# gunesevitan/otto-multi-objective-recommender-system

Hardware: AMD Instinct MI355X
Metric: aid-pairs/sec covisitation build (higher is better)
Workload: dtype u64

## Files before the change

otto-multi-objective-recommender-system_amd/csrc/otto_covis.hip:

```cpp
#include "common.h"
#include "topk.h"
#include "scan.h"
#include "../../include/otto_covis.h"

#include <stdarg.h>
#include <string.h>
#include <type_traits>
#include <vector>

namespace otto {

static thread_local std::string g_err;
void set_error(const char* fmt, ...) {
    char buf[1024];
    va_list ap;
    va_start(ap, fmt);
    vsnprintf(buf, sizeof buf, fmt, ap);
    va_end(ap);
    g_err = buf;
}

struct WinPairs {
    const int64_t* off;
    int W;
// ... 1015 lines not shown
                wave_topk_push(best[j], lb, k);
            }
        }
    }
}

template <int NW, int GATHER_U, typename FB>
__device__ __forceinline__ void for_each_record_batch(const uint64_t* sorted_desc, const uint32_t* rec, uint64_t r0, uint64_t r1,
                                                      int wid, FB fb) {
    const unsigned lane = lane_id();
    const uint32_t l = lane & 31u;
    const int half = (int)(lane >> 5);
    if (r0 >= r1) return;
    auto load_desc = [&](uint64_t cb) {
        const uint64_t mine = cb + (uint64_t)lane * NW + wid;
        return mine < r1 ? sorted_desc[mine] : 0ull;
    };
    uint64_t d = load_desc(r0);
    for (uint64_t cb = r0; cb < r1; cb += (uint64_t)NW * 64) {
        const uint64_t cbn = cb + (uint64_t)NW * 64;
        const uint64_t dn = cbn < r1 ? load_desc(cbn) : 0ull;
        const uint64_t left = r1 - cb;
        const int nrun = left >= (uint64_t)NW * 64 ? 64 : (int)((left + NW - 1 - wid) / NW);
        uint32_t rcA[GATHER_U], rcB[GATHER_U];
        uint64_t slA[GATHER_U], slB[GATHER_U];
        bool okA[GATHER_U], okB[GATHER_U];
        auto issue = [&](int t, uint32_t (&rc)[GATHER_U], uint64_t (&sl)[GATHER_U], bool (&ok)[GATHER_U]) {
#pragma unroll
            for (int u = 0; u < GATHER_U; ++u) {
                const int src = t + 2 * u + half;
                const uint64_t dd = (uint64_t)__shfl((unsigned long long)d, src & 63, 64);
                const uint32_t sp = desc_sp(dd);
                const uint64_t s0 = desc_slot(dd);
                ok[u] = src < 64 && l < desc_len(dd) && l != sp;
                rc[u] = ok[u] ? rec[s0 + l] : 0u;
                sl[u] = s0 + (sp != DESC_SP_NONE ? sp : l);
            }
        };
        auto consume = [&](uint32_t (&rc)[GATHER_U], uint64_t (&sl)[GATHER_U], bool (&ok)[GATHER_U]) { fb(rc, sl, ok); };
        if (nrun > 0) issue(0, rcA, slA, okA);
        for (int t = 0; t < nrun; t += 4 * GATHER_U) {
            const bool hasB = t + 2 * GATHER_U < nrun;
            if (hasB) issue(t + 2 * GATHER_U, rcB, slB, okB);
            consume(rcA, slA, okA);
            if (t + 4 * GATHER_U < nrun) issue(t + 4 * GATHER_U, rcA, slA, okA);
            if (hasB) consume(rcB, slB, okB);
        }
        d = dn;
    }
}

template <int NW, int GATHER_U, bool NEED_SL, typename FB>
__device__ __forceinline__ void for_each_record_seg(const uint64_t* sorted_desc, const uint32_t* rec, uint64_t r0, uint64_t r1,
                                                    int wid, uint8_t* s_seg, FB fb, const uint64_t* d0p = nullptr) {
    const unsigned lane = lane_id();
    const uint32_t g = lane >> 3, gl4 = (lane & 7u) << 2;
    if (r0 >= r1) return;
    auto load_desc = [&](uint64_t cb) {
        const uint64_t mine = cb + (uint64_t)lane * NW + wid;
        return mine < r1 ? sorted_desc[mine] : 0ull;
    };
    uint64_t d = d0p ? *d0p : load_desc(r0);
    for (uint64_t cb = r0; cb < r1; cb += (uint64_t)NW * 64) {
        const uint64_t cbn = cb + (uint64_t)NW * 64;
        const uint64_t dn = cbn < r1 ? load_desc(cbn) : 0ull;
        const uint32_t len = desc_len(d);
        const uint32_t segs = (len + 7u) >> 3;
        const uint32_t incl = wave_incl_scan(segs), excl = incl - segs;
        const uint32_t total = (uint32_t)__builtin_amdgcn_readlane((int)incl, 63);
#pragma unroll
        for (uint32_t k = 0; k < 4; ++k)
            if (k < segs) s_seg[excl + k] = (uint8_t)((lane << 2) | k);
        wave_lds_sync();
        const int nstep = (int)((total + 7u) >> 3);
        const uint64_t recb = (uint64_t)(uintptr_t)rec;
        const uint64_t pre = (recb + (desc_slot(d) << 2)) | ((uint64_t)desc_len(d) << 50) | ((uint64_t)desc_sp(d) << 58);
        const int plo = (int)(uint32_t)pre, phi = (int)(uint32_t)(pre >> 32);
        uint32_t rcA[GATHER_U], rcB[GATHER_U];
        uint64_t slA[NEED_SL ? GATHER_U : 1], slB[NEED_SL ? GATHER_U : 1];
        uint64_t okA[GATHER_U], okB[GATHER_U];
        constexpr int ICMP_NE = 33, ICMP_ULT = 36, ICMP_SLT = 40;
        auto issue = [&](int t, uint32_t (&rc)[GATHER_U], uint64_t (&sl)[NEED_SL ? GATHER_U : 1], uint64_t (&ok)[GATHER_U]) {
            const uint32_t qb = (uint32_t)t * 8u + g;
            const int lim = (int)total - 8 * t;
#pragma unroll
            for (int u = 0; u < GATHER_U; ++u) {
                const uint32_t r = (uint32_t)s_seg[qb + 8u * u];
                const int src = (int)(r & 0xFCu);
                const uint32_t lo = (uint32_t)__builtin_amdgcn_ds_bpermute(src, plo);
                const uint32_t hi = (uint32_t)__builtin_amdgcn_ds_bpermute(src, phi);
                const uint32_t off4 = ((r & 3u) << 5) | gl4;
                const uint32_t len4 = (hi >> 16) & 0xFFu, sp4 = hi >> 24;
                const uint64_t base = ((uint64_t)(hi & 0xFFFFu) << 32) | lo;
                if (NEED_SL) sl[NEED_SL ? u : 0] = (base - recb + (sp4 != DESC_SP_NONE * 4u ? sp4 : off4)) >> 2;
                ok[u] = __builtin_amdgcn_sicmp((int)g, lim - 8 * u, ICMP_SLT) & __builtin_amdgcn_uicmp(off4, len4, ICMP_ULT) &
                        __builtin_amdgcn_uicmp(off4, sp4, ICMP_NE);
                rc[u] = *reinterpret_cast<const __attribute__((address_space(1))) uint32_t*>((uintptr_t)(base + off4));
            }
        };
        if (nstep > 0) issue(0, rcA, slA, okA);
        for (int t = 0; t < nstep; t += 2 * GATHER_U) {
            const bool hasB = t + GATHER_U < nstep;
            if (hasB) issue(t + GATHER_U, rcB, slB, okB);
            fb(rcA, slA, okA);
            if (t + 2 * GATHER_U < nstep) issue(t + 2 * GATHER_U, rcA, slA, okA);
            if (hasB) fb(rcB, slB, okB);
        }
        wave_lds_sync();
        d = dn;
    }
}

template <int NW, int GATHER_U, typename F>
__device__ __forceinline__ void for_each_record(const uint64_t* sorted_desc, const uint32_t* rec, uint64_t r0, uint64_t r1,
                                                int wid, F f) {
    for_each_record_batch<NW, GATHER_U>(sorted_desc, rec, r0, r1, wid,
                                        [&](uint32_t (&rc)[GATHER_U], uint64_t (&sl)[GATHER_U], bool (&ok)[GATHER_U]) {
#pragma unroll
        for (int u = 0; u < GATHER_U; ++u)
            if (ok[u]) f(rc[u], sl[u]);
    });
}

__device__ __forceinline__ uint32_t rec_hash(uint32_t rc) { return (rc & REC_AID_MASK) * 0x9E3779B1u; }

struct PartArgs {
    const uint64_t* chunks;
    uint32_t n_chunks;
    const uint64_t* cnt64;
    const uint8_t* boost;
    const uint64_t* run_start;
    const uint64_t* sorted_desc;
    const uint32_t* rec;
    const uint32_t* tw;
    const uint64_t* litem_start;
    uint32_t* pcount;
    uint32_t* pcursor;
    const uint64_t* pstart;
    uint32_t* prec;
    uint32_t* ptw;
    uint32_t l_cap;
    int window_max;
    int allow_packed;
    uint32_t* flag;
    uint32_t* ovf_count;
    uint32_t* work;
};

__host__ __device__ __forceinline__ uint64_t bucket_cap(uint64_t n_records, int lgR) {
    return lgR == 0 ? 0ull : 2ull * ((n_records + (1ull << lgR) - 1ull) >> lgR) + 256ull;
}
struct ItemCap {
    const uint64_t* items;
// ... 343 lines not shown
            ord[r] = (uint32_t)s;
            for (uint64_t p = 1; p < items; ++p) ord[a.n_pilots[mode] + sm + p - r - 1] = (uint32_t)(s + p);
            const uint64_t cs = run[9] + ex_c;
            for (uint64_t q = 0; q < nch; ++q) a.chunks[cs + q] = (uint64_t)x | (q << 26);
        }
        run[0] += tot_small & 0xFFF;
        run[1] += (tot_small >> 12) & 0xFFF;
        run[2] += tot_l;
#pragma unroll
        for (int m = 0; m < 3; ++m) {
            run[6 + m] += (tot_small >> (24 + 12 * m)) & 0xFFF;
            run[3 + m] += tot_m[m];
        }
        run[9] += tot_c;
    }
}

constexpr uint64_t TAB_EMPTY = ~0ull;

struct ItemDesc {
    uint32_t it;
    uint64_t item;
    uint64_t rb, re;
    uint64_t ps, pe;
};

#ifdef OTTO_PHASE_PROF
#define OTTO_PH(i) do { if (threadIdx.x == 0) { const unsigned long long _t = clock64(); ph[i] += _t - ph_t; ph_t = _t; } } while (0)
#else
#define OTTO_PH(i) do {} while (0)
#endif
template <int LOG2T, int THREADS, int GROUP, bool PACKED, int MINW, int GU, int INS_CH, bool DBG>
__global__ __launch_bounds__(THREADS, MINW) void k_reduce(ReduceArgs a) {
    constexpr int T = 1 << LOG2T;
    constexpr int NW = THREADS / 64;
    constexpr bool TP = GROUP == OTTO_COVIS_GROUP_TIME && PACKED;
    using K = typename std::conditional<GROUP == OTTO_COVIS_GROUP_TIME && !PACKED, KeyW, KeyN>::type;
    constexpr bool WIDE = GROUP == OTTO_COVIS_GROUP_TIME && !PACKED;
    auto kw = [](K key) -> uint64_t { if constexpr (TP) return key.c >> REC_AID_BITS; else return kweight(key); };
    constexpr bool DYNAMIC = true;
    constexpr int EXCAP = 64;
    constexpr int PKD = GROUP == OTTO_COVIS_GROUP_TIME ? 1 : PK;
    constexpr bool BOUND = GROUP == OTTO_COVIS_GROUP_TYPE && PKD > 1 && NW == 1;
    constexpr int CCAP = 256;
    constexpr bool HOT = NW > 1 && GROUP == OTTO_COVIS_GROUP_TYPE;
    __shared__ uint64_t s_tab[PACKED ? T : 1];
    __shared__ uint32_t s_key[PACKED ? 1 : T];
    __shared__ uint32_t s_v[3][PACKED ? 1 : T];
    constexpr int OCAP = NW == 1 ? 1 : (LOG2T == 12 ? 1920 : (LOG2T == 14 ? 10240 : (THREADS == 512 ? 4608 : 6144)));
    constexpr int RCAP = OCAP / NW;
    __shared__ uint16_t s_occ[OCAP];
    __shared__ uint32_t s_wcnt[NW];
    __shared__ uint32_t s_hcnt[NW];
    __shared__ uint16_t s_lbi[NW > 1 ? PKD : 1][NW > 1 ? THREADS : 1];
    __shared__ uint64_t s_exw[(NW > 1 || BOUND) ? PKD : 1][(NW > 1 || BOUND) ? EXCAP : 1];
    __shared__ uint16_t s_cand[BOUND ? CCAP : 1];
    __shared__ uint32_t s_exy[1][(NW > 1 && WIDE) ? EXCAP : 1];
    __shared__ uint64_t s_thrw[PK];
    __shared__ uint32_t s_thry[PK];
    __shared__ uint32_t s_nex[PK];
    __shared__ uint32_t s_more;
    __shared__ uint32_t s_ovf;
    constexpr int LISTCAP = BOUND ? S_CAP : 256;
    __shared__ uint16_t s_list[NW == 1 ? LISTCAP : 1];
    __shared__ uint8_t s_seg[NW * 256 + 32];
    __shared__ ItemDesc s_cur;
    __shared__ ItemDesc s_nxt;

    const int wid = threadIdx.x >> 6;
    const unsigned lane = lane_id();
#ifdef OTTO_PHASE_PROF
    unsigned long long ph[16] = {0, 0, 0, 0, 0, 0, 0, 0, 0, 0, 0, 0, 0, 0, 0, 0}, ph_t = clock64();
#endif

    auto fetch_item = [&](uint32_t idx, ItemDesc& d) {
        d.it = 0xFFFFFFFFu;
        d.item = 0ull;
        if (idx < a.n_work) {
            d.it = a.order ? a.order[idx] : idx;
            d.item = a.items[d.it];
        }
    };
    auto fetch_ranges = [&](ItemDesc& d) {
        d.rb = d.re = d.ps = d.pe = 0;
        if (d.it != 0xFFFFFFFFu) {
            const uint32_t xx = (uint32_t)(d.item & REC_AID_MASK);
            d.rb = a.run_start[xx];
            d.re = a.run_start[xx + 1];
            if ((d.item >> 50) != 0 && a.pstart) {
                d.ps = a.pstart[d.it];
                const uint64_t cap = a.pstart[d.it + 1] - d.ps, got = a.pcursor[d.it];
                d.pe = d.ps + (got < cap ? got : cap);
            }
        }
    };
    ItemDesc cur, nx;
    uint32_t idx_next = 0, idx_far = 0;
    constexpr uint32_t DQ = THREADS == S_THREADS ? 16 : 4;
    uint32_t pool = 0, pool_end = 0, pool_next = 0;
    auto take = [&]() {
        const uint32_t r = pool++;
        if (pool == pool_end) {
            pool = pool_next;
            pool_end = pool + DQ;
            pool_next = atomicAdd(a.work_counter, DQ);
        }
        return r;
    };
    if (DYNAMIC) {
        if (threadIdx.x == 0) {
            pool = atomicAdd(a.work_counter, 2 * DQ);
            pool_end = pool + DQ;
            pool_next = pool + DQ;
            const uint32_t i0 = take();
            idx_next = take();
            idx_far = take();
            fetch_item(i0, cur);
            fetch_ranges(cur);
            s_cur = cur;
        }
    } else {
        fetch_item(blockIdx.x, cur);
        fetch_ranges(cur);
    }
    uint32_t sidx = blockIdx.x;
    auto clear_slot = [&](int i) {
        if (PACKED) {
            s_tab[PACKED ? i : 0] = TAB_EMPTY;
        } else {
            s_key[PACKED ? 0 : i] = KEY_EMPTY;
            s_v[0][PACKED ? 0 : i] = 0; s_v[1][PACKED ? 0 : i] = 0; s_v[2][PACKED ? 0 : i] = 0;
        }
    };
    auto clear_table = [&]() {
        for (int i = threadIdx.x; i < T; i += THREADS) clear_slot(i);
    };
    if (NW > 1) {
        clear_table();
        if (threadIdx.x == 0) s_ovf = 0;
    }
    constexpr int BU = GROUP == OTTO_COVIS_GROUP_TIME ? 4 : ((PACKED && THREADS == L_THREADS) ? 12 : 6);
    constexpr bool PREF = THREADS == L_THREADS && GROUP != OTTO_COVIS_GROUP_TIME;
    constexpr bool WARM = (THREADS == L_THREADS || THREADS == 512) && GROUP != OTTO_COVIS_GROUP_TIME;
    uint32_t pre[PREF ? BU : 1];
    bool pre_valid = false;
    auto prefetch_next = [&]() {
        if (!PREF) return;
        const uint64_t nitem = s_nxt.item;
        pre_valid = s_nxt.it != 0xFFFFFFFFu && (nitem >> 50) != 0 && a.pstart != nullptr;
        if (!pre_valid) return;
        const uint64_t ps = s_nxt.ps, pe = s_nxt.pe;
#pragma unroll
        for (int u = 0; u < (PREF ? BU : 1); ++u) {
            const uint64_t i = ps + threadIdx.x + (uint64_t)u * THREADS;
            pre[u] = i < pe ? a.prec[i] : KEY_EMPTY;
        }
    };

    for (;;) {
        if (DYNAMIC) {
            __syncthreads();
            cur = s_cur;
        }
        if (cur.it == 0xFFFFFFFFu) break;
        OTTO_PH(0);
        const uint32_t it = cur.it;
        if (DYNAMIC) {
            if (threadIdx.x == 0) fetch_item(idx_next, nx);
#ifdef OTTO_PHASE_PROF
            if (threadIdx.x == 0) { const unsigned long long _t = clock64(); ph[13] += _t - ph_t; }
#endif
        } else {
            fetch_item(sidx + gridDim.x, nx);
        }
        const uint64_t item = cur.item;
        const uint32_t x = (uint32_t)(item & REC_AID_MASK);
        const uint32_t part = (uint32_t)((item >> 26) & 0xFFFFFFu);
        constexpr bool CAN_PART = THREADS != M_THREADS;
        const int lgR = CAN_PART ? (int)(item >> 50) : 0;
        const uint32_t pmask = (1u << lgR) - 1u;
        const int pshift = 32 - LOG2T - lgR;

        K guess[PKD];
        const bool use_guess = NW > 1 && lgR > 0 && a.tau_w != nullptr;
#pragma unroll
        for (int j = 0; j < PKD; ++j) {
            kclear(guess[j]);
            if (use_guess && j < (BOUND ? 1 : a.nk)) {
                const size_t o = (size_t)j * a.n_aids + x;
                kload(guess[j], a.tau_w[o], WIDE ? a.tau_y[o] : 0u);
            }
        }
        if (NW == 1 && !(DBG && (a.debug_skip & 4))) clear_table();
        if (NW == 1) {
            s_ovf = 0;
            wave_lds_sync();
        }
        OTTO_PH(1);

        auto probe_step = [&](uint32_t y) -> uint32_t { return (((y * 0x85EBCA6Bu) ^ (y >> 7)) * 0xC2B2AE35u >> (32 - LOG2T)) | 1u; };
        uint32_t wc = 0;
        auto note_new = [&](uint64_t m, uint32_t slot) {
            if (NW == 1) return;
            if (m == 0) return;
            const uint32_t pos = wc + __builtin_amdgcn_mbcnt_hi((uint32_t)(m >> 32), __builtin_amdgcn_mbcnt_lo((uint32_t)m, 0u));
            if (__builtin_amdgcn_inverse_ballot_w64(m) && pos < (uint32_t)RCAP) s_occ[NW > 1 ? wid * RCAP + pos : 0] = (uint16_t)slot;
            wc += (uint32_t)__popcll(m);
        };
        constexpr int ICMP_EQ = 32, ICMP_NE = 33;
        auto probe_on = [&](uint32_t y, uint32_t slot, unsigned long long add, unsigned long long fresh) -> uint32_t {
            const uint32_t step = probe_step(y);
            for (int probe = 1; probe < T; ++probe) {
                slot = (slot + step) & (T - 1);
                const unsigned long long old = atomicCAS((unsigned long long*)&s_tab[PACKED ? slot : 0], (unsigned long long)TAB_EMPTY, fresh | add);
                if (old == TAB_EMPTY) return slot;
                if ((uint32_t)(old >> 36) == y) {
                    atomicAdd((unsigned long long*)&s_tab[PACKED ? slot : 0], add);
                    return 0xFFFFFFFFu;
                }
            }
            s_ovf = 1;
// ... 95 lines not shown
                    uint32_t sl = rec_hash(r) >> (32 - LOG2T);
                    uint32_t late = 0xFFFFFFFFu;
                    if (ok[q]) {
                        bool found = old[q] == KEY_EMPTY || old[q] == y;
                        const uint32_t step = probe_step(y);
                        for (int probe = 1; !found && probe < T; ++probe) {
                            sl = (sl + step) & (T - 1);
                            const uint32_t o2 = atomicCAS(&s_key[PACKED ? 0 : sl], KEY_EMPTY, y);
                            if (o2 == KEY_EMPTY) late = sl;
                            found = o2 == KEY_EMPTY || o2 == y;
                        }
                        if (!found) s_ovf = 1;
                        else wide_add(r, sl, e[c0 + q < N ? c0 + q : 0]);
                    }
                    note_new(__builtin_amdgcn_uicmp(late, 0xFFFFFFFFu, ICMP_NE), late);
                }
            }
        };

        auto slot_keys = [&](int i, K (&out)[PKD]) {
            uint32_t y, v0, v1, v2;
            if (PACKED) {
                const uint64_t v = s_tab[i];
                y = v == TAB_EMPTY ? KEY_EMPTY : (uint32_t)(v >> 36);
                v0 = (uint32_t)v & 0xFFFu; v1 = (uint32_t)(v >> 12) & 0xFFFu; v2 = (uint32_t)(v >> 24) & 0xFFFu;
            } else {
                y = s_key[i];
                v0 = s_v[0][i]; v1 = s_v[1][i]; v2 = s_v[2][i];
            }
#pragma unroll
            for (int j = 0; j < PKD; ++j) {
                uint64_t uw = 0, qw = 0;
                if (y != KEY_EMPTY) {
                    if (TP) uw = (uint64_t)v0 | ((uint64_t)v1 << 12) | ((uint64_t)v2 << 24);
                    else if (GROUP == OTTO_COVIS_GROUP_TIME) qw = 65536ull * v0 + (((uint64_t)v2 << 32) | v1);
                    else if (PACKED) uw = __umul24(v0, a.coef[j][0]) + __umul24(v1, a.coef[j][1]) + __umul24(v2, a.coef[j][2]);
                    else uw = (uint64_t)v0 * a.coef[j][0] + (uint64_t)v1 * a.coef[j][1] + (uint64_t)v2 * a.coef[j][2];
                }
                kmake(out[j], uw, qw, y);
            }
        };
        auto emit = [&](int j, K best) {
            const bool valid = (int)lane < a.k && kvalid(best);
            if (lgR == 0) {
                const size_t o = ((size_t)(a.kind_base + j) * a.n_aids + x) * (size_t)a.k + lane;
                if (valid) { a.out_y[o] = kaid(best); a.out_w[o] = kw(best); }
                const int nvalid = __popcll(__ballot(valid));
                if (lane == 0) a.out_n[(size_t)(a.kind_base + j) * a.n_aids + x] = nvalid;
            } else if ((int)lane < a.k) {
                const size_t o = ((size_t)it * a.nk + j) * (size_t)a.k + lane;
                kstore(best, &a.part_w[o], &a.part_y[o]);
            }
        };
        if (DBG && (a.debug_skip & 1)) {
        } else if (lgR > 0 && a.pstart) {
            const uint64_t ps = cur.ps, pe = cur.pe;
            bool first = true;
            for (uint64_t i0 = ps + threadIdx.x; i0 < pe; i0 += BU * THREADS) {
                uint32_t rc[BU], e[BU];
                if (PREF && first && pre_valid) {
#pragma unroll
                    for (int u = 0; u < BU; ++u) { rc[u] = pre[PREF ? u : 0]; e[u] = 0u; }
                } else {
#pragma unroll
                    for (int u = 0; u < BU; ++u) {
                        const uint64_t i = i0 + (uint64_t)u * THREADS;
                        rc[u] = i < pe ? a.prec[i] : KEY_EMPTY;
                        e[u] = (GROUP == OTTO_COVIS_GROUP_TIME && i < pe) ? a.ptw[i] : 0u;
                    }
                }
                first = false;
#ifdef OTTO_PHASE_PROF
                asm volatile("s_waitcnt vmcnt(0)" ::: "memory");
                if (threadIdx.x == 0) { const unsigned long long _t = clock64(); ph[12] += _t - ph_t; ph[2] -= _t - ph_t; }
#endif
                uint64_t okb[BU];
#pragma unroll
                for (int u = 0; u < BU; ++u) okb[u] = __ballot(rc[u] != KEY_EMPTY);
                insert_batch(std::integral_constant<int, BU>{}, rc, okb, e);
                if (s_ovf) break;
            }
        } else {
            constexpr bool NEED_SL = GROUP == OTTO_COVIS_GROUP_TIME;
            for_each_record_seg<NW, GU, NEED_SL>(a.sorted_desc, a.rec, cur.rb, cur.re, wid, s_seg + wid * 256,
                                                 [&](uint32_t (&rc)[GU], uint64_t (&sl)[NEED_SL ? GU : 1], uint64_t (&ok)[GU]) {
                uint32_t e[GU];
                uint64_t okb[GU];
#pragma unroll
                for (int u = 0; u < GU; ++u) {
                    okb[u] = ok[u];
                    if (lgR != 0) okb[u] &= __ballot(((rec_hash(rc[u]) >> pshift) & pmask) == part);
                    e[u] = (GROUP == OTTO_COVIS_GROUP_TIME && __builtin_amdgcn_inverse_ballot_w64(okb[u])) ? a.tw[sl[NEED_SL ? u : 0]] : 0u;
                }
                insert_batch(std::integral_constant<int, GU>{}, rc, okb, e);
            });
        }
        if (NW > 1 && lane == 0) s_wcnt[NW > 1 ? wid : 0] = wc;
        pre_valid = false;
        if (!DYNAMIC || threadIdx.x == 0) fetch_ranges(nx);
        OTTO_PH(2);
        __syncthreads();
        OTTO_PH(3);
        const bool ovf = s_ovf != 0;
        if constexpr (BOUND) {
        if (ovf) {
            if (threadIdx.x == 0) {
                a.flag[x] = 1;
                a.boost[x] = (uint8_t)(lgR - l_log2r(a.cnt64[x], 0, a.l_cap, a.allow_packed) + 1);
                atomicAdd(a.ovf_count, 1u);
            }
        } else if (!(DBG && (a.debug_skip & 2))) {
            constexpr int MPL = T / THREADS;
            uint32_t lo0 = a.coef[0][0], lo1 = a.coef[0][1], lo2 = a.coef[0][2], hi0 = lo0, hi1 = lo1, hi2 = lo2;
            for (int j = 1; j < a.nk; ++j) {
                lo0 = min(lo0, a.coef[j][0]); lo1 = min(lo1, a.coef[j][1]); lo2 = min(lo2, a.coef[j][2]);
                hi0 = max(hi0, a.coef[j][0]); hi1 = max(hi1, a.coef[j][1]); hi2 = max(hi2, a.coef[j][2]);
            }
            auto slot_read = [&](int i, uint32_t& y, uint32_t& v0, uint32_t& v1, uint32_t& v2) {
                if (PACKED) {
                    const uint64_t v = s_tab[PACKED ? i : 0];
                    y = v == TAB_EMPTY ? KEY_EMPTY : (uint32_t)(v >> 36);
                    v0 = (uint32_t)v & 0xFFFu; v1 = (uint32_t)(v >> 12) & 0xFFFu; v2 = (uint32_t)(v >> 24) & 0xFFFu;
                } else {
                    y = s_key[PACKED ? 0 : i];
                    v0 = s_v[0][PACKED ? 0 : i]; v1 = s_v[1][PACKED ? 0 : i]; v2 = s_v[2][PACKED ? 0 : i];
                }
            };
            auto weight = [&](uint32_t v0, uint32_t v1, uint32_t v2, uint32_t c0, uint32_t c1, uint32_t c2) -> uint64_t {
                if (PACKED) return (uint64_t)(__umul24(v0, c0) + __umul24(v1, c1) + __umul24(v2, c2));
                return (uint64_t)v0 * c0 + (uint64_t)v1 * c1 + (uint64_t)v2 * c2;
            };
            auto slot_lohi = [&](int i, K& kl, K& kh) {
                uint32_t y, v0, v1, v2;
                slot_read(i, y, v0, v1, v2);
                const bool valid = y != KEY_EMPTY;
                kmake(kl, valid ? weight(v0, v1, v2, lo0, lo1, lo2) : 0ull, 0ull, y);
                kmake(kh, valid ? weight(v0, v1, v2, hi0, hi1, hi2) : 0ull, 0ull, y);
            };
            auto slot_kind_key = [&](int i, int j) {
                uint32_t y, v0, v1, v2;
                slot_read(i, y, v0, v1, v2);
                K key;
                kmake(key, y != KEY_EMPTY ? weight(v0, v1, v2, a.coef[j][0], a.coef[j][1], a.coef[j][2]) : 0ull, 0ull, y);
                return key;
            };
            auto emit_ranked = [&](int j, K key, uint32_t rank, int nv) {
                const bool put = kvalid(key) && rank < (uint32_t)a.k;
                if (lgR == 0) {
                    const size_t o = ((size_t)(a.kind_base + j) * a.n_aids + x) * (size_t)a.k + rank;
                    if (put) { a.out_y[o] = kaid(key); a.out_w[o] = kw(key); }
                    if (lane == 0) a.out_n[(size_t)(a.kind_base + j) * a.n_aids + x] = nv < a.k ? nv : a.k;
                } else {
// ... 348 lines not shown
                K lb;
                kclear(lb);
                int bi = -1;
                for (int w = 0; w < nreg; ++w) {
                    const int total = dense ? (int)(hot ? s_hcnt[NW > 1 ? w : 0] : s_wcnt[NW > 1 ? w : 0]) : T;
                    for (int i = (int)lane; i < total; i += 64) {
                        const int sl = dense ? (int)s_occ[NW > 1 ? w * RCAP + i : 0] : i;
                        const K key = slot_key1(sl, c0, c1, c2);
                        if (kbetter(key, lb)) { lb = key; bi = sl; }
                    }
                }
                K best = lb;
                wave_bitonic_sort_desc(best);
                for (int w = 0; w < nreg; ++w) {
                    const int total = dense ? (int)(hot ? s_hcnt[NW > 1 ? w : 0] : s_wcnt[NW > 1 ? w : 0]) : T;
                    for (int i0 = 0; i0 < total; i0 += 64) {
                        const int i = i0 + (int)lane;
                        K key;
                        kclear(key);
                        if (i < total) {
                            const int sl = dense ? (int)s_occ[NW > 1 ? w * RCAP + i : 0] : i;
                            if (sl != bi) key = slot_key1(sl, c0, c1, c2);
                        }
                        wave_topk_push(best, key, a.k);
                    }
                }
                emit(j, best);
            };
            auto append = [&](int j, K key) {
                const uint32_t pos = atomicAdd(&s_nex[j], 1u);
                if (pos < (uint32_t)EXCAP) kstore(key, &s_exw[j][pos], &s_exy[0][WIDE ? pos : 0]);
                else s_more = 1;
            };

            bool fast_done = false;
            bool pre_issued = false;
            constexpr bool SH = HOT && NW <= 4;
            constexpr int SHR = 4;
            if (SH && hot && a.hot_ok >= 2) {
                __syncthreads();
                uint32_t pre[NW + 1];
                pre[0] = 0;
#pragma unroll
                for (int w = 0; w < NW; ++w) pre[w + 1] = pre[w] + s_hcnt[NW > 1 ? w : 0];
                const uint32_t th = pre[NW];
                if (th < (uint32_t)a.k) {
                    hot = false;
                    nwalk = nocc;
                    nit = (int)((nwalk + 63u) / 64u);
                } else if (th <= 64u * SHR) {
#ifdef OTTO_PHASE_PROF
                    if (threadIdx.x == 0) ph[14]++;
#endif
                    if (wid < a.nk && wid < PKD) {
                        const int j = wid;
                        const uint32_t c0 = a.coef[j][0], c1 = a.coef[j][1], c2 = a.coef[j][2];
                        K keys[SHR], lbk;
                        kclear(lbk);
#pragma unroll
                        for (int q = 0; q < SHR; ++q) {
                            const uint32_t e = (uint32_t)q * 64u + lane;
                            kclear(keys[q]);
                            if (e < th) {
                                int w = 0;
#pragma unroll
                                for (int ww = 1; ww < NW; ++ww)
                                    if (e >= pre[ww]) w = ww;
                                const uint32_t sl = s_occ[NW > 1 ? w * RCAP + (int)(e - pre[w]) : 0];
                                keys[q] = slot_key1((int)sl, c0, c1, c2);
                                if (kbetter(keys[q], lbk)) lbk = keys[q];
                            }
                        }
                        kstore(lbk, &s_exw[j][lane], &s_exy[0][WIDE ? lane : 0]);
                        wave_lds_sync();
                        uint32_t rank = 0;
#pragma unroll 8
                        for (int i = 0; i < 64; ++i) {
                            K o;
                            kload(o, s_exw[j][i], s_exy[0][WIDE ? i : 0]);
                            kcount_better(rank, o, lbk);
                        }
                        const uint64_t mk = __ballot(kvalid(lbk) && rank == (uint32_t)(a.k - 1));
                        K thr;
                        kclear(thr);
                        if (mk) thr = kshfl(lbk, __ffsll((unsigned long long)mk) - 1);
                        wave_lds_sync();
                        uint32_t n = 0;
#pragma unroll
                        for (int q = 0; q < SHR; ++q) {
                            const bool c = kvalid(keys[q]) && !kbetter(thr, keys[q]);
                            const uint64_t m = __ballot(c);
                            const uint32_t pos = n + __builtin_amdgcn_mbcnt_hi((uint32_t)(m >> 32), __builtin_amdgcn_mbcnt_lo((uint32_t)m, 0u));
                            if (c && pos < (uint32_t)EXCAP) kstore(keys[q], &s_exw[j][pos], &s_exy[0][WIDE ? pos : 0]);
                            n += (uint32_t)__popcll(m);
                        }
                        wave_lds_sync();
                        if (n > (uint32_t)EXCAP) wave_exact_topk(j);
                        else finish_list(j, n, false);
                    }
                    fast_done = true;
                }
            }
            bool gv = use_guess && !fast_done;
#pragma unroll
            for (int j = 0; j < PKD; ++j)
                if (j < a.nk && !kvalid(guess[j])) gv = false;
            if (gv) {
                if (threadIdx.x < PK) s_nex[threadIdx.x] = 0;
                if (threadIdx.x == 0) { s_more = 0; if (WARM) s_nxt = nx; }
                __syncthreads();
                uint32_t warm = 0;
                if (WARM && s_nxt.it != 0xFFFFFFFFu && (s_nxt.item >> 50) != 0 && a.pstart != nullptr) {
                    const uint64_t wi = s_nxt.ps + (uint64_t)threadIdx.x * 16u;
                    if (wi < s_nxt.pe) warm = a.prec[wi];
                }
                for (int q = 0; q < nit; ++q) {
                    const int sl = slot_at(q);
                    if (sl < 0) continue;
                    K kk[PKD];
                    slot_keys(sl, kk);
#pragma unroll
                    for (int j = 0; j < PKD; ++j)
                        if (j < a.nk && kvalid(kk[j]) && kbetter(kk[j], guess[j])) append(j, kk[j]);
                }
                asm volatile("" :: "v"(warm));
                __syncthreads();
                prefetch_next();
                pre_issued = true;
                bool ok = s_more == 0;
#pragma unroll
                for (int j = 0; j < PKD; ++j)
                    if (j < a.nk && s_nex[j] < (uint32_t)a.k) ok = false;
#ifdef OTTO_PHASE_PROF
                if (threadIdx.x == 0) { ph[8]++; if (ok) ph[9]++; else if (s_more) ph[11]++; else ph[10]++; }
#endif
                if (ok) {
                    if (wid < a.nk && wid < PKD) finish_list(wid, s_nex[wid], true);
                    fast_done = true;
                }
                __syncthreads();
            }
            OTTO_PH(7);
            if (!fast_done) {
                K lb[PKD];
                int bi[PKD];
                constexpr int NCK = (PACKED && THREADS <= 512) ? 3 : 0;
                K ck[NCK > 0 ? NCK : 1][PKD];
                for (;;) {
#pragma unroll
                for (int j = 0; j < PKD; ++j) { kclear(lb[j]); bi[j] = 0xFFFF; }
#pragma unroll
                for (int q = 0; q < NCK; ++q) {
                    const int sl = q < nit ? slot_at(q) : -1;
#pragma unroll
                    for (int j = 0; j < PKD; ++j) kclear(ck[q][j]);
                    if (sl >= 0) {
                        slot_keys(sl, ck[q]);
#pragma unroll
                        for (int j = 0; j < PKD; ++j)
                            if (kbetter(ck[q][j], lb[j])) { lb[j] = ck[q][j]; bi[j] = sl; }
                    }
                }
                for (int q = NCK; q < nit; ++q) {
                    const int sl = slot_at(q);
                    if (sl < 0) continue;
                    K kk[PKD];
                    slot_keys(sl, kk);
#pragma unroll
                    for (int j = 0; j < PKD; ++j)
                        if (kbetter(kk[j], lb[j])) { lb[j] = kk[j]; bi[j] = sl; }
                }
#pragma unroll
                for (int j = 0; j < PKD; ++j)
                    if (j < a.nk) s_lbi[j][NW > 1 ? threadIdx.x : 0] = (uint16_t)bi[j];
                if (threadIdx.x < PK) s_nex[threadIdx.x] = 0;
                if (threadIdx.x == 0) s_more = 0;
                __syncthreads();
                if (hot) {
                    uint32_t th = 0;
#pragma unroll
                    for (int w = 0; w < NW; ++w) th += s_hcnt[NW > 1 ? w : 0];
                    if (th < (uint32_t)a.k) {
                        hot = false;
                        nwalk = nocc;
                        nit = (int)((nwalk + 63u) / 64u);
                        continue;
                    }
                }
                break;
                }
                OTTO_PH(4);
                if (wid < a.nk && wid < PKD) {
                    K gb;
                    kclear(gb);
                    const uint32_t c0 = a.coef[wid][0], c1 = a.coef[wid][1], c2 = a.coef[wid][2];
#pragma unroll
                    for (int q = 0; q < NW; ++q) {
                        const uint32_t sl = s_lbi[wid][NW > 1 ? q * 64 + lane : 0];
                        if (sl != 0xFFFFu) {
                            const K o = slot_key1((int)sl, c0, c1, c2);
                            if (kbetter(o, gb)) gb = o;
                        }
                    }
                    kstore(gb, &s_exw[wid][lane], &s_exy[0][WIDE ? lane : 0]);
                    wave_lds_sync();
                    uint32_t rank = 0;
#pragma unroll 8
                    for (int i = 0; i < 64; ++i) {
                        K o;
                        kload(o, s_exw[wid][i], s_exy[0][WIDE ? i : 0]);
                        kcount_better(rank, o, gb);
                    }
                    const uint64_t mk = __ballot(kvalid(gb) && rank == (uint32_t)(a.k - 1));
                    K thr;
                    kclear(thr);
                    if (mk) thr = kshfl(gb, __ffsll((unsigned long long)mk) - 1);
                    if (lane == 0) kstore(thr, &s_thrw[wid], &s_thry[wid]);
                    if (use_guess && kvalid(gb) && rank == 31u) ktau_store(gb, a.tau_w, a.tau_y, (size_t)wid * a.n_aids + x);
                    wave_lds_sync();
                }
                OTTO_PH(5);
                __syncthreads();
                K thr[PKD];
#pragma unroll
                for (int j = 0; j < PKD; ++j) kload(thr[j], s_thrw[j], s_thry[j]);
#pragma unroll
                for (int q = 0; q < NCK; ++q) {
#pragma unroll
                    for (int j = 0; j < PKD; ++j)
                        if (j < a.nk && kvalid(ck[q][j]) && !kbetter(thr[j], ck[q][j])) append(j, ck[q][j]);
                }
                for (int q = NCK; q < nit; ++q) {
                    const int sl = slot_at(q);
                    if (sl < 0) continue;
                    K kk[PKD];
                    slot_keys(sl, kk);
#pragma unroll
                    for (int j = 0; j < PKD; ++j)
                        if (j < a.nk && kvalid(kk[j]) && !kbetter(thr[j], kk[j])) append(j, kk[j]);
                }
                if (PREF && !pre_issued && threadIdx.x == 0) s_nxt = nx;
                __syncthreads();
                if (!pre_issued) prefetch_next();
                OTTO_PH(6);
                if (wid < a.nk && wid < PKD) {
                    if (s_more) wave_exact_topk(wid);
                    else finish_list(wid, s_nex[wid] < (uint32_t)EXCAP ? s_nex[wid] : (uint32_t)EXCAP, false);
                }
                OTTO_PH(7);
            }
        }
        __syncthreads();
        if (!(DBG && (a.debug_skip & 4))) {
            if (dense) {
                for (uint32_t idx = lane; idx < nocc; idx += 64u) clear_slot((int)s_occ[NW > 1 ? wid * RCAP + idx : 0]);
            } else {
                clear_table();
            }
        }
        if (threadIdx.x == 0) s_ovf = 0;
        }

        if (DYNAMIC) {
            __syncthreads();
            if (threadIdx.x == 0) {
                s_cur = nx;
                idx_next = idx_far;
                idx_far = take();
            }
        } else {
            cur = nx;
            sidx += gridDim.x;
        }
    }
#ifdef OTTO_PHASE_PROF
    if (threadIdx.x == 0 && a.prof)
        for (int i = 0; i < 16; ++i) atomicAdd(&a.prof[i], ph[i]);
#endif
}

template <typename K, bool RAW>
__device__ __forceinline__ void merge_lists(const ReduceArgs& a, uint32_t it, uint32_t x, int lgR, int j, unsigned lane) {
    const uint64_t ncand = (uint64_t)a.k << lgR;
    auto fetch = [&](uint64_t c0) {
        const uint64_t c = c0 + lane;
        K cand;
        kclear(cand);
        if (c < ncand) {
            const size_t o = ((size_t)(it + c / a.k) * a.nk + j) * (size_t)a.k + (c % a.k);
            kload(cand, a.part_w[o], a.part_y[o]);
        }
        return cand;
    };
    K best;
    kclear(best);
    K cand = fetch(0);
    for (uint64_t c0 = 0; c0 < ncand; c0 += 64) {
        const K nxt = c0 + 64 < ncand ? fetch(c0 + 64) : cand;
        if (c0 == 0) { best = cand; wave_bitonic_sort_desc(best); }
        else wave_topk_push(best, cand, a.k);
        cand = nxt;
    }
    const bool valid = (int)lane < a.k && kvalid(best);
    const size_t o = ((size_t)(a.kind_base + j) * a.n_aids + x) * (size_t)a.k + lane;
    if (valid) {
        a.out_y[o] = kaid(best);
        if constexpr (RAW) a.out_w[o] = best.c >> REC_AID_BITS;
        else a.out_w[o] = kweight(best);
    }
    const int nvalid = __popcll(__ballot(valid));
    if (lane == 0) a.out_n[(size_t)(a.kind_base + j) * a.n_aids + x] = nvalid;
}

template <int GROUP>
__global__ __launch_bounds__(64 * PK) void k_merge(ReduceArgs a) {
    const uint32_t it = blockIdx.x;
    if (it >= a.n_items) return;
    const uint64_t item = a.items[it];
    const uint32_t part = (uint32_t)((item >> 26) & 0xFFFFFFu);
    const int lgR = (int)(item >> 50);
    if (part != 0 || lgR == 0) return;
    const uint32_t x = (uint32_t)(item & REC_AID_MASK);
    if (a.flag[x]) return;
    const unsigned lane = lane_id();
    const int j = (int)(threadIdx.x >> 6);
    if (j >= a.nk) return;
    if constexpr (GROUP == OTTO_COVIS_GROUP_TIME) {
        if (heavy_mode(a.cnt64[x], a.allow_packed, a.l_cap) != 0) merge_lists<KeyN, true>(a, it, x, lgR, j, lane);
        else merge_lists<KeyW, false>(a, it, x, lgR, j, lane);
    } else {
// ... 640 lines not shown
    OTTO_TRY(c->pcursor.ensure((size_t)a.n_items * 4, 0, s));
    OTTO_TRY(c->pstart.ensure((size_t)(a.n_items + 1) * 8, 0, s));
    OTTO_TRY(c->partial.ensure(scan_partial_bytes((int64_t)a.n_items), 0, s));
    OTTO_HIP(hipMemsetAsync(c->pcursor.p, 0, (size_t)a.n_items * 4, s));
    PartArgs pa{c->chunks.as<uint64_t>(), (uint32_t)c->n_chunks, c->cnt64.as<uint64_t>(), c->boost.as<uint8_t>(),
                c->run_start.as<uint64_t>(), c->sorted_desc.as<uint64_t>(), c->rec.as<uint32_t>(), c->tw.as<uint32_t>(),
                c->litem_start.as<uint64_t>(), c->pcount.as<uint32_t>(), c->pcursor.as<uint32_t>(),
                c->pstart.as<uint64_t>(), nullptr, nullptr, c->l_cap, c->p.window, a.allow_packed, c->flag.as<uint32_t>(),
                c->counters.as<uint32_t>()};
    const uint32_t pres = 256u * 4u;
    const uint32_t pgrid = (uint32_t)(c->n_chunks < pres ? c->n_chunks : pres);
    const uint32_t cgrid = (uint32_t)(c->n_chunks < 256u * 8u ? c->n_chunks : 256u * 8u);
    const bool sized = c->part_sized && !c->exact_round;
    if (sized) {
        kname(c, OTTO_COVIS_T_PARTITION, "k_partition<true>");
        OTTO_TRY(device_scan(ItemCap{a.items, c->cnt64.as<uint64_t>()}, (int64_t)a.n_items, c->pstart.as<uint64_t>(), c->partial.as<uint64_t>(), s));
    } else {
        kname(c, OTTO_COVIS_T_PARTITION, "k_partition<false> + k_partition<true>");
        OTTO_HIP(hipMemsetAsync(c->pcount.p, 0, (size_t)a.n_items * 4, s));
        k_partition<false, false><<<cgrid, 256, 0, s>>>(pa);
        OTTO_HIP(hipGetLastError());
        OTTO_TRY(device_scan(PCount{c->pcount.as<uint32_t>()}, (int64_t)a.n_items, c->pstart.as<uint64_t>(), c->partial.as<uint64_t>(), s));
    }
    uint64_t bucket_total = 0;
    OTTO_HIP(hipMemcpyAsync(&bucket_total, c->pstart.as<uint64_t>() + a.n_items, 8, hipMemcpyDeviceToHost, s));
    OTTO_HIP(hipStreamSynchronize(s));
    OTTO_TRY(c->prec.ensure((size_t)(bucket_total ? bucket_total : 1) * 4, 0, s));
    if (time) OTTO_TRY(c->ptw.ensure((size_t)(bucket_total ? bucket_total : 1) * 4, 0, s));
    pa.prec = c->prec.as<uint32_t>();
    pa.ptw = time ? c->ptw.as<uint32_t>() : nullptr;
    pa.work = c->counters.as<uint32_t>() + 8;
    OTTO_HIP(hipMemsetAsync(pa.work, 0, 4, s));
    if (time) k_partition<true, true><<<pgrid, 256, 0, s>>>(pa);
    else k_partition<true, false><<<pgrid, 256, 0, s>>>(pa);
    OTTO_HIP(hipGetLastError());
    tend(c, OTTO_COVIS_T_PARTITION, s);
    return 0;
}

template <int GROUP>
static int launch_reduce(otto_covis_ctx* c, ReduceArgs a, int bin, hipStream_t s) {
    a.items = c->items[bin].as<uint64_t>();
    a.n_items = (uint32_t)c->n_items[bin];
    a.n_work = a.n_items;
    if (a.n_items == 0) return 0;
    a.order = nullptr;
    a.allow_packed = c->items_allow_packed > 0 ? c->items_allow_packed : 0;
    uint32_t* wc = c->counters.as<uint32_t>() + 1 + bin;
    OTTO_HIP(hipMemsetAsync(wc, 0, 4, s));
    a.work_counter = wc;
#ifdef OTTO_PHASE_PROF
    static unsigned long long* d_prof = nullptr;
    static hipEvent_t pe0 = nullptr, pe1 = nullptr;
    if (!d_prof) { OTTO_HIP(hipMalloc(&d_prof, 128)); OTTO_HIP(hipEventCreate(&pe0)); OTTO_HIP(hipEventCreate(&pe1)); }
    a.prof = d_prof;
    auto prof_begin = [&]() { (void)hipMemsetAsync(d_prof, 0, 128, s); (void)hipEventRecord(pe0, s); };
    auto prof_end = [&](const char* tag, uint32_t n_work) {
        unsigned long long h[16];
        (void)hipEventRecord(pe1, s); (void)hipStreamSynchronize(s); (void)hipMemcpy(h, d_prof, 128, hipMemcpyDeviceToHost);
        float ms = 0.f; (void)hipEventElapsedTime(&ms, pe0, pe1);
        unsigned long long tot = 0; for (int i = 0; i < 8; ++i) tot += h[i];
        fprintf(stderr, "[phase-prof] %s items %u  %.3f ms:", tag, n_work, ms);
        for (int i = 0; i < 8; ++i) fprintf(stderr, " p%d %.1f%%", i, tot ? 100.0 * h[i] / tot : 0.0);
        fprintf(stderr, "  (ticks %llu) guess: tried %llu ok %llu toofew %llu overflow %llu | record wait (not in p2): %.1f%%, next-item fetch (in p1): %.1f%% of the ticks | single-wave selection of few heavy keys: %llu items\n", tot, h[8], h[9], h[10], h[11], tot ? 100.0 * (double)h[12] / tot : 0.0, tot ? 100.0 * (double)h[13] / tot : 0.0, h[14]);
    };
#else
    auto prof_begin = [&]() {};
    auto prof_end = [&](const char*, uint32_t) {};
#endif
    if (bin == 0) {
        const uint32_t s_res = 256u * (uint32_t)c->s_wgs;
        uint32_t grid = a.n_items < s_res ? a.n_items : s_res;
        tbegin(c, OTTO_COVIS_T_REDUCE_S, s);
        prof_begin();
        OTTO_LAUNCH_REDUCE(OTTO_COVIS_T_REDUCE_S, grid, S_THREADS, a, S_LOG2T, S_THREADS, GROUP, true, 5, 4);
        prof_end("S", a.n_work);
        tend(c, OTTO_COVIS_T_REDUCE_S, s);
    } else if (bin == 1) {
        uint32_t grid = a.n_items < 256u * 4u ? a.n_items : 256u * 4u;
        tbegin(c, OTTO_COVIS_T_REDUCE_M, s);
        prof_begin();
        OTTO_LAUNCH_REDUCE(OTTO_COVIS_T_REDUCE_M, grid, M_THREADS, a, M_LOG2T, M_THREADS, GROUP, true, 4, 4);
        prof_end("M", a.n_work);
        tend(c, OTTO_COVIS_T_REDUCE_M, s);
    } else {
        a.pstart = nullptr;
        if (c->partition && c->n_chunks) {
            if (c->part_gen == c->items_gen && !c->exact_round && (GROUP != OTTO_COVIS_GROUP_TIME || c->part_has_tw)) {
            } else {
                const bool with_tw = c->p.want_time;
                c->part_gen = 0;
                OTTO_TRY(run_partition(c, a, with_tw, s));
                if (!c->exact_round) { c->part_gen = c->items_gen; c->part_has_tw = with_tw; }
            }
            a.pstart = c->pstart.as<uint64_t>();
            a.pcursor = c->pcursor.as<uint32_t>();
            a.prec = c->prec.as<uint32_t>();
            a.ptw = c->ptw.as<uint32_t>();
        }
        tbegin(c, OTTO_COVIS_T_REDUCE_L, s);
        for (int mode = 2; mode >= 0; --mode) {
            if (!c->n_order[mode]) continue;
            ReduceArgs am = a;
            am.order = c->lorder[mode].as<uint32_t>();
            am.n_work = (uint32_t)c->n_order[mode];
            OTTO_HIP(hipMemsetAsync(wc, 0, 4, s));
            prof_begin();
            if (mode == 2) {
                const uint32_t grid = am.n_work < 256u * 2u ? am.n_work : 256u * 2u;
                OTTO_LAUNCH_REDUCE(OTTO_COVIS_T_REDUCE_L, grid, 512, am, L_LOG2T, 512, GROUP, true, 4, 4);
            } else if (mode == 1) {
                const uint32_t grid = am.n_work < 256u ? am.n_work : 256u;
                OTTO_LAUNCH_REDUCE(OTTO_COVIS_T_REDUCE_L, grid, L_THREADS, am, LP_LOG2T, L_THREADS, GROUP, true, 4, 2);
            } else {
                const uint32_t grid = am.n_work < 256u ? am.n_work : 256u;
                OTTO_LAUNCH_REDUCE(OTTO_COVIS_T_REDUCE_L, grid, L_THREADS, am, L_LOG2T, L_THREADS, GROUP, false, 4, 2);
            }
// ... 411 lines not shown
```

Baseline: 59.75 billion.

## Move item prefetch to last wave, warm next item's records, reduce bounds in-wave

For the M-bin kernel, next-item fetching and queue management move from thread 0 to the first lane of the last wave. That wave is otherwise idle during per-key selection, and it now issues warm-up loads of the next item's descriptors and first and last records so they are cached. For packed tables, the per-thread lower bounds are reduced with wave shuffles and written straight into s_exw, which drops the s_lbi slot array and the slot_key recomputation. Profiling counters for gather waits, clear time and selection time are also added behind a compile-time flag. The extra warm loads use memory bandwidth and may bring no benefit when the items are small.

```diff
diff --git a/otto-multi-objective-recommender-system_amd/csrc/otto_covis.hip b/otto-multi-objective-recommender-system_amd/csrc/otto_covis.hip
--- a/otto-multi-objective-recommender-system_amd/csrc/otto_covis.hip
+++ b/otto-multi-objective-recommender-system_amd/csrc/otto_covis.hip
@@ -1091,15 +1091,25 @@
 
 template <int NW, int GATHER_U, bool NEED_SL, typename FB>
 __device__ __forceinline__ void for_each_record_seg(const uint64_t* sorted_desc, const uint32_t* rec, uint64_t r0, uint64_t r1,
-                                                    int wid, uint8_t* s_seg, FB fb, const uint64_t* d0p = nullptr) {
+                                                    int wid, uint8_t* s_seg, FB fb, const uint64_t* d0p = nullptr,
+                                                    unsigned long long* pw = nullptr) {
     const unsigned lane = lane_id();
     const uint32_t g = lane >> 3, gl4 = (lane & 7u) << 2;
     if (r0 >= r1) return;
+#ifdef OTTO_PHASE_PROF
+    unsigned long long pw_t = clock64();
+#else
+    (void)pw;
+#endif
     auto load_desc = [&](uint64_t cb) {
         const uint64_t mine = cb + (uint64_t)lane * NW + wid;
         return mine < r1 ? sorted_desc[mine] : 0ull;
     };
     uint64_t d = d0p ? *d0p : load_desc(r0);
+#ifdef OTTO_PHASE_PROF
+    asm volatile("s_waitcnt vmcnt(0)" ::: "memory");
+    if (pw) { const unsigned long long _t = clock64(); pw[0] += _t - pw_t; }
+#endif
     for (uint64_t cb = r0; cb < r1; cb += (uint64_t)NW * 64) {
         const uint64_t cbn = cb + (uint64_t)NW * 64;
         const uint64_t dn = cbn < r1 ? load_desc(cbn) : 0ull;
@@ -1138,6 +1148,13 @@
             }
         };
         if (nstep > 0) issue(0, rcA, slA, okA);
+#ifdef OTTO_PHASE_PROF
+        if (pw && cb == r0) {
+            pw_t = clock64();
+            asm volatile("s_waitcnt vmcnt(0)" ::: "memory");
+            pw[1] += clock64() - pw_t;
+        }
+#endif
         for (int t = 0; t < nstep; t += 2 * GATHER_U) {
             const bool hasB = t + GATHER_U < nstep;
             if (hasB) issue(t + GATHER_U, rcB, slB, okB);
@@ -1587,7 +1604,8 @@
     __shared__ uint16_t s_occ[OCAP];
     __shared__ uint32_t s_wcnt[NW];
     __shared__ uint32_t s_hcnt[NW];
-    __shared__ uint16_t s_lbi[NW > 1 ? PKD : 1][NW > 1 ? THREADS : 1];
+    constexpr bool INWAVE = PACKED;
+    __shared__ uint16_t s_lbi[(NW > 1 && !INWAVE) ? PKD : 1][(NW > 1 && !INWAVE) ? THREADS : 1];
     __shared__ uint64_t s_exw[(NW > 1 || BOUND) ? PKD : 1][(NW > 1 || BOUND) ? EXCAP : 1];
     __shared__ uint16_t s_cand[BOUND ? CCAP : 1];
     __shared__ uint32_t s_exy[1][(NW > 1 && WIDE) ? EXCAP : 1];
@@ -1604,8 +1622,11 @@
 
     const int wid = threadIdx.x >> 6;
     const unsigned lane = lane_id();
+    constexpr bool HANDOVER = THREADS == M_THREADS;
+    const int swid = HANDOVER ? __builtin_amdgcn_readfirstlane(wid) : wid;
+    const bool pipe = threadIdx.x == (HANDOVER ? (NW - 1) * 64 : 0);
 #ifdef OTTO_PHASE_PROF
-    unsigned long long ph[16] = {0, 0, 0, 0, 0, 0, 0, 0, 0, 0, 0, 0, 0, 0, 0, 0}, ph_t = clock64();
+    unsigned long long ph[24] = {0, 0, 0, 0, 0, 0, 0, 0, 0, 0, 0, 0, 0, 0, 0, 0, 0, 0, 0, 0, 0, 0, 0, 0}, ph_t = clock64();
 #endif
 
     auto fetch_item = [&](uint32_t idx, ItemDesc& d) {
@@ -1643,7 +1664,7 @@
         return r;
     };
     if (DYNAMIC) {
-        if (threadIdx.x == 0) {
+        if (pipe) {
             pool = atomicAdd(a.work_counter, 2 * DQ);
             pool_end = pool + DQ;
             pool_next = pool + DQ;
@@ -1701,7 +1722,7 @@
         OTTO_PH(0);
         const uint32_t it = cur.it;
         if (DYNAMIC) {
-            if (threadIdx.x == 0) fetch_item(idx_next, nx);
+            if (pipe) fetch_item(idx_next, nx);
 #ifdef OTTO_PHASE_PROF
             if (threadIdx.x == 0) { const unsigned long long _t = clock64(); ph[13] += _t - ph_t; }
 #endif
@@ -1903,6 +1924,33 @@
                 kstore(best, &a.part_w[o], &a.part_y[o]);
             }
         };
+        constexpr int WARM_B = 4;
+        auto warm_next = [&]() {
+            if (!HANDOVER) return;
+            auto bc = [&](uint64_t v) -> uint64_t {
+                return ((uint64_t)(uint32_t)__builtin_amdgcn_readfirstlane((int)(uint32_t)(v >> 32)) << 32) |
+                       (uint32_t)__builtin_amdgcn_readfirstlane((int)(uint32_t)v);
+            };
+            if ((uint32_t)__builtin_amdgcn_readfirstlane((int)nx.it) == 0xFFFFFFFFu) return;
+            const uint64_t rb = bc(nx.rb), re = bc(nx.re);
+            uint64_t d[WARM_B];
+#pragma unroll
+            for (int b = 0; b < WARM_B; ++b) {
+                const uint64_t r = rb + (uint64_t)(b * 64 + (int)lane);
+                d[b] = r < re ? a.sorted_desc[r] : 0ull;
+            }
+            uint32_t acc = 0;
+#pragma unroll
+            for (int b = 0; b < WARM_B; ++b) {
+                const uint32_t len = desc_len(d[b]);
+                if (len) {
+                    const uint64_t s0 = desc_slot(d[b]);
+                    acc |= a.rec[s0] | a.rec[s0 + len - 1u];
+                }
+            }
+            asm volatile("" :: "v"(acc));
+        };
+        const int nsel = a.nk < PKD ? a.nk : PKD;
         if (DBG && (a.debug_skip & 1)) {
         } else if (lgR > 0 && a.pstart) {
             const uint64_t ps = cur.ps, pe = cur.pe;
@@ -1944,11 +1992,15 @@
                     e[u] = (GROUP == OTTO_COVIS_GROUP_TIME && __builtin_amdgcn_inverse_ballot_w64(okb[u])) ? a.tw[sl[NEED_SL ? u : 0]] : 0u;
                 }
                 insert_batch(std::integral_constant<int, GU>{}, rc, okb, e);
-            });
+            }
+#ifdef OTTO_PHASE_PROF
+            , nullptr, threadIdx.x == 0 ? &ph[15] : nullptr
+#endif
+            );
         }
         if (NW > 1 && lane == 0) s_wcnt[NW > 1 ? wid : 0] = wc;
         pre_valid = false;
-        if (!DYNAMIC || threadIdx.x == 0) fetch_ranges(nx);
+        if (!DYNAMIC || pipe) fetch_ranges(nx);
         OTTO_PH(2);
         __syncthreads();
         OTTO_PH(3);
@@ -2403,8 +2455,11 @@
 #ifdef OTTO_PHASE_PROF
                     if (threadIdx.x == 0) ph[14]++;
 #endif
-                    if (wid < a.nk && wid < PKD) {
-                        const int j = wid;
+#ifdef OTTO_PHASE_PROF
+                    const unsigned long long sel_t = clock64();
+#endif
+                    if (swid < nsel) {
+                        const int j = swid;
                         const uint32_t c0 = a.coef[j][0], c1 = a.coef[j][1], c2 = a.coef[j][2];
                         K keys[SHR], lbk;
                         kclear(lbk);
@@ -2448,7 +2503,12 @@
                         wave_lds_sync();
                         if (n > (uint32_t)EXCAP) wave_exact_topk(j);
                         else finish_list(j, n, false);
+                    } else if (swid == NW - 1) {
+                        warm_next();
                     }
+#ifdef OTTO_PHASE_PROF
+                    if (threadIdx.x == 0) ph[18] += clock64() - sel_t;
+#endif
                     fast_done = true;
                 }
             }
@@ -2458,7 +2518,8 @@
                 if (j < a.nk && !kvalid(guess[j])) gv = false;
             if (gv) {
                 if (threadIdx.x < PK) s_nex[threadIdx.x] = 0;
-                if (threadIdx.x == 0) { s_more = 0; if (WARM) s_nxt = nx; }
+                if (threadIdx.x == 0) s_more = 0;
+                if (WARM && pipe) s_nxt = nx;
                 __syncthreads();
                 uint32_t warm = 0;
                 if (WARM && s_nxt.it != 0xFFFFFFFFu && (s_nxt.item >> 50) != 0 && a.pstart != nullptr) {
@@ -2486,7 +2547,13 @@
                 if (threadIdx.x == 0) { ph[8]++; if (ok) ph[9]++; else if (s_more) ph[11]++; else ph[10]++; }
 #endif
                 if (ok) {
+#ifdef OTTO_PHASE_PROF
+                    const unsigned long long sel_t = clock64();
+#endif
                     if (wid < a.nk && wid < PKD) finish_list(wid, s_nex[wid], true);
+#ifdef OTTO_PHASE_PROF
+                    if (threadIdx.x == 0) ph[18] += clock64() - sel_t;
+#endif
                     fast_done = true;
                 }
                 __syncthreads();
@@ -2522,8 +2589,22 @@
                         if (kbetter(kk[j], lb[j])) { lb[j] = kk[j]; bi[j] = sl; }
                 }
 #pragma unroll
-                for (int j = 0; j < PKD; ++j)
-                    if (j < a.nk) s_lbi[j][NW > 1 ? threadIdx.x : 0] = (uint16_t)bi[j];
+                for (int j = 0; j < PKD; ++j) {
+                    if (!INWAVE) {
+                        if (j < a.nk) s_lbi[!INWAVE ? j : 0][(NW > 1 && !INWAVE) ? threadIdx.x : 0] = (uint16_t)bi[j];
+                        continue;
+                    }
+                    K g = lb[j];
+#pragma unroll
+                    for (int m = 1; m < NW; m <<= 1) {
+                        const K o = kshfl_xor(g, m);
+                        if (kbetter(o, g)) g = o;
+                    }
+                    if (j < a.nk && (lane & (NW - 1)) == 0) {
+                        const int gi = wid * (64 / NW) + (int)(lane / NW);
+                        kstore(g, &s_exw[j][gi], &s_exy[0][WIDE ? gi : 0]);
+                    }
+                }
                 if (threadIdx.x < PK) s_nex[threadIdx.x] = 0;
                 if (threadIdx.x == 0) s_more = 0;
                 __syncthreads();
@@ -2541,33 +2622,40 @@
                 break;
                 }
                 OTTO_PH(4);
-                if (wid < a.nk && wid < PKD) {
+                if (swid >= nsel) {
+                    if (swid == NW - 1) warm_next();
+                } else {
+                    const int j = swid;
                     K gb;
-                    kclear(gb);
-                    const uint32_t c0 = a.coef[wid][0], c1 = a.coef[wid][1], c2 = a.coef[wid][2];
-#pragma unroll
-                    for (int q = 0; q < NW; ++q) {
-                        const uint32_t sl = s_lbi[wid][NW > 1 ? q * 64 + lane : 0];
-                        if (sl != 0xFFFFu) {
-                            const K o = slot_key1((int)sl, c0, c1, c2);
-                            if (kbetter(o, gb)) gb = o;
+                    if (INWAVE) {
+                        kload(gb, s_exw[j][lane], s_exy[0][WIDE ? lane : 0]);
+                    } else {
+                        kclear(gb);
+                        const uint32_t c0 = a.coef[j][0], c1 = a.coef[j][1], c2 = a.coef[j][2];
+#pragma unroll
+                        for (int q = 0; q < NW; ++q) {
+                            const uint32_t sl = s_lbi[!INWAVE ? j : 0][(NW > 1 && !INWAVE) ? q * 64 + lane : 0];
+                            if (sl != 0xFFFFu) {
+                                const K o = slot_key1((int)sl, c0, c1, c2);
+                                if (kbetter(o, gb)) gb = o;
+                            }
                         }
+                        kstore(gb, &s_exw[j][lane], &s_exy[0][WIDE ? lane : 0]);
+                        wave_lds_sync();
                     }
-                    kstore(gb, &s_exw[wid][lane], &s_exy[0][WIDE ? lane : 0]);
-                    wave_lds_sync();
                     uint32_t rank = 0;
 #pragma unroll 8
                     for (int i = 0; i < 64; ++i) {
                         K o;
-                        kload(o, s_exw[wid][i], s_exy[0][WIDE ? i : 0]);
+                        kload(o, s_exw[j][i], s_exy[0][WIDE ? i : 0]);
                         kcount_better(rank, o, gb);
                     }
                     const uint64_t mk = __ballot(kvalid(gb) && rank == (uint32_t)(a.k - 1));
                     K thr;
                     kclear(thr);
                     if (mk) thr = kshfl(gb, __ffsll((unsigned long long)mk) - 1);
-                    if (lane == 0) kstore(thr, &s_thrw[wid], &s_thry[wid]);
-                    if (use_guess && kvalid(gb) && rank == 31u) ktau_store(gb, a.tau_w, a.tau_y, (size_t)wid * a.n_aids + x);
+                    if (lane == 0) kstore(thr, &s_thrw[j], &s_thry[j]);
+                    if (use_guess && kvalid(gb) && rank == 31u) ktau_store(gb, a.tau_w, a.tau_y, (size_t)j * a.n_aids + x);
                     wave_lds_sync();
                 }
                 OTTO_PH(5);
@@ -2590,7 +2678,7 @@
                     for (int j = 0; j < PKD; ++j)
                         if (j < a.nk && kvalid(kk[j]) && !kbetter(thr[j], kk[j])) append(j, kk[j]);
                 }
-                if (PREF && !pre_issued && threadIdx.x == 0) s_nxt = nx;
+                if (PREF && !pre_issued && pipe) s_nxt = nx;
                 __syncthreads();
                 if (!pre_issued) prefetch_next();
                 OTTO_PH(6);
@@ -2602,6 +2690,9 @@
             }
         }
         __syncthreads();
+#ifdef OTTO_PHASE_PROF
+        const unsigned long long clr_t = clock64();
+#endif
         if (!(DBG && (a.debug_skip & 4))) {
             if (dense) {
                 for (uint32_t idx = lane; idx < nocc; idx += 64u) clear_slot((int)s_occ[NW > 1 ? wid * RCAP + idx : 0]);
@@ -2610,11 +2701,14 @@
             }
         }
         if (threadIdx.x == 0) s_ovf = 0;
+#ifdef OTTO_PHASE_PROF
+        if (threadIdx.x == 0) ph[17] += clock64() - clr_t;
+#endif
         }
 
         if (DYNAMIC) {
             __syncthreads();
-            if (threadIdx.x == 0) {
+            if (pipe) {
                 s_cur = nx;
                 idx_next = idx_far;
                 idx_far = take();
@@ -2626,7 +2720,7 @@
     }
 #ifdef OTTO_PHASE_PROF
     if (threadIdx.x == 0 && a.prof)
-        for (int i = 0; i < 16; ++i) atomicAdd(&a.prof[i], ph[i]);
+        for (int i = 0; i < 24; ++i) atomicAdd(&a.prof[i], ph[i]);
 #endif
 }
 
@@ -3373,17 +3467,18 @@
 #ifdef OTTO_PHASE_PROF
     static unsigned long long* d_prof = nullptr;
     static hipEvent_t pe0 = nullptr, pe1 = nullptr;
-    if (!d_prof) { OTTO_HIP(hipMalloc(&d_prof, 128)); OTTO_HIP(hipEventCreate(&pe0)); OTTO_HIP(hipEventCreate(&pe1)); }
+    if (!d_prof) { OTTO_HIP(hipMalloc(&d_prof, 192)); OTTO_HIP(hipEventCreate(&pe0)); OTTO_HIP(hipEventCreate(&pe1)); }
     a.prof = d_prof;
-    auto prof_begin = [&]() { (void)hipMemsetAsync(d_prof, 0, 128, s); (void)hipEventRecord(pe0, s); };
+    auto prof_begin = [&]() { (void)hipMemsetAsync(d_prof, 0, 192, s); (void)hipEventRecord(pe0, s); };
     auto prof_end = [&](const char* tag, uint32_t n_work) {
-        unsigned long long h[16];
-        (void)hipEventRecord(pe1, s); (void)hipStreamSynchronize(s); (void)hipMemcpy(h, d_prof, 128, hipMemcpyDeviceToHost);
+        unsigned long long h[24];
+        (void)hipEventRecord(pe1, s); (void)hipStreamSynchronize(s); (void)hipMemcpy(h, d_prof, 192, hipMemcpyDeviceToHost);
         float ms = 0.f; (void)hipEventElapsedTime(&ms, pe0, pe1);
         unsigned long long tot = 0; for (int i = 0; i < 8; ++i) tot += h[i];
         fprintf(stderr, "[phase-prof] %s items %u  %.3f ms:", tag, n_work, ms);
         for (int i = 0; i < 8; ++i) fprintf(stderr, " p%d %.1f%%", i, tot ? 100.0 * h[i] / tot : 0.0);
-        fprintf(stderr, "  (ticks %llu) guess: tried %llu ok %llu toofew %llu overflow %llu | record wait (not in p2): %.1f%%, next-item fetch (in p1): %.1f%% of the ticks | single-wave selection of few heavy keys: %llu items\n", tot, h[8], h[9], h[10], h[11], tot ? 100.0 * (double)h[12] / tot : 0.0, tot ? 100.0 * (double)h[13] / tot : 0.0, h[14]);
+        fprintf(stderr, "  (ticks %llu) guess: tried %llu ok %llu toofew %llu overflow %llu | record wait (not in p2): %.1f%%, next-item fetch (in p1): %.1f%% of the ticks | single-wave selection of few heavy keys: %llu items | gather: descriptor wait %.1f%%, first-record wait %.1f%% (both in p2) | clear %.1f%% (in p0) | single-wave select / finish_list %.1f%% (in p7)\n", tot, h[8], h[9], h[10], h[11], tot ? 100.0 * (double)h[12] / tot : 0.0, tot ? 100.0 * (double)h[13] / tot : 0.0, h[14],
+                tot ? 100.0 * (double)h[15] / tot : 0.0, tot ? 100.0 * (double)h[16] / tot : 0.0, tot ? 100.0 * (double)h[17] / tot : 0.0, tot ? 100.0 * (double)h[18] / tot : 0.0);
     };
 #else
     auto prof_begin = [&]() {};
```

New measurement: 61.06 billion (median of 6 runs). +2.2%, better.
